# zsyOAOA/ResShift

Measured on AMD Instinct MI355X. Metric: images/sec (1x3x64x64 LR -> 3x256x256, 15-step ResShift sampling loop incl. VQ encode/decode), higher is better.
Workload: dtype f16x2 encoder + UNet (hi+lo fp16 pairs, 3 MFMAs per product: fp32-class) + f16 decoder (parity policy); 1 GPU; realsr_swinunet_realesrgan256: batch 32/GPU x 1 GPU, 1x3x64x64 LR -> 3x256x256, 15 steps, random-init weights; precision_policy=parity, parallelism=dp1 (batch sharded, one RCCL weight broadcast, no data-path collective)

## Files before the change

resshift_amd/csrc/ops.hip:

```cpp
#include "launchers.h"
#include "weight_pack.h"
#include <algorithm>
#include <cmath>
#include <cstdio>
#include <cstdlib>
#include <vector>

extern "C" {

static void* dev_copy(const void* host, size_t bytes) {
    void* d = nullptr;
    if (hipMalloc(&d, bytes) != hipSuccess) return nullptr;
    (void)hipMemcpy(d, host, bytes, hipMemcpyHostToDevice);
    return d;
}
static void* frag_major_from_device_rows(const void* wdev, int N, int K, int ld, int lo_off) {
    std::vector<f16> rows((size_t)N * ld), out((size_t)N * K * (lo_off >= 0 ? 2 : 1));
    if (hipMemcpy(rows.data(), wdev, rows.size() * sizeof(f16), hipMemcpyDeviceToHost) != hipSuccess) return nullptr;
    frag_major_fill(N, K, out.data(), lo_off >= 0, [&](int n, int k) { return rows[(size_t)n * ld + k]; },
                    [&](int n, int k) { return rows[(size_t)n * ld + (lo_off >= 0 ? lo_off : 0) + k]; });
    return dev_copy(out.data(), out.size() * sizeof(f16));
}
static void* pack_rows_dev(const float* w_ref_host, int Cout, int Cin, int taps, int prec) {
    std::vector<char> o((size_t)Cout * taps * Cin * rs_dtype_size(prec));
    if (prec == RS_F16) rs_pack_rows_f16(w_ref_host, Cout, Cin, taps, Cin, (f16*)o.data());
    else if (prec == RS_F16S) rs_pack_rows_split(w_ref_host, Cout, Cin, taps, Cin, (f16*)o.data());
    else rs_pack_rows_f32(w_ref_host, Cout, Cin, taps, Cin, (float*)o.data());
    return dev_copy(o.data(), o.size());
}
static void bias_tables_dev(const float* table_host, int heads, float** bias_t, float** bias_n, float** bias_c) {
    std::vector<float> bt(bias_t ? (size_t)heads * 4096 : 0), bn(bias_n ? (size_t)heads * 4096 : 0), bc(bias_c ? (size_t)heads * 256 : 0);
    rs_pack_bias_tables(table_host, heads, bias_t ? bt.data() : nullptr, bias_n ? bn.data() : nullptr);
    if (bias_c) rs_pack_bias_compact(table_host, heads, bc.data());
    if (bias_t) *bias_t = (float*)dev_copy(bt.data(), bt.size() * 4);
    if (bias_n) *bias_n = (float*)dev_copy(bn.data(), bn.size() * 4);
    if (bias_c) *bias_c = (float*)dev_copy(bc.data(), bc.size() * 4);
}

static int time_launches(const IGemmParams& p, int in_prec, int out_prec, const ConvPlan& pl, int reps, hipStream_t st, float* ms_out) {
    int rc = 0;
    hipEvent_t e0, e1;
    (void)hipEventCreate(&e0); (void)hipEventCreate(&e1);
    (void)hipEventRecord(e0, st);
    for (int i = 0; i < reps; ++i) rc |= rs_conv_launch(&p, in_prec, out_prec, 1, &pl, st);
    (void)hipEventRecord(e1, st);
    (void)hipEventSynchronize(e1);
    float ms = 0.f;
    (void)hipEventElapsedTime(&ms, e0, e1);
    if (ms_out) *ms_out = ms / (float)std::max(1, reps);
    (void)hipEventDestroy(e0); (void)hipEventDestroy(e1);
    return rc;
}

static int op_conv_run(IGemmParams p, int in_prec, int out_prec, hipStream_t st, bool halo_only = false, bool timed = false, int reps = 0, float* ms_out = nullptr) {
    ConvPlan pl{};
    (void)rs_conv_plan(&p, in_prec, out_prec, 1, &pl);
    if (halo_only && pl.kernel != CK_HALO && pl.kernel != CK_HALO_SEG) return rs_set_last_error("shape is not eligible for the halo kernel", -1);
    float* part = nullptr;
    if (pl.splitk > 1) { (void)hipMalloc((void**)&part, (size_t)pl.splitk * p.M * p.Cout * sizeof(float)); p.partial = part; }
    int rc = rs_conv_launch(&p, in_prec, out_prec, 1, &pl, st);
    if (rc) rs_set_last_error("igemm launch rejected the shape", -1);
    else if (timed) rc = time_launches(p, in_prec, out_prec, pl, reps, st, ms_out);
    (void)hipStreamSynchronize(st);
    if (part) (void)hipFree(part);
    return rc;
}

int rs_op_conv2d(const void* x0, const void* x1, const float* w_ref_host, const float* bias_host, const void* res, void* y, int B, int Hs,
                 int Ws, int C0, int C1, int Cout, int KH, int KW, int stride, int pad_t, int pad_l, int Ho, int Wo, int up, int act,
                 int in_prec, int out_prec, int force_direct, void* stream) {
    hipStream_t st = (hipStream_t)stream;
    const int Cin = C0 + C1;
    const size_t K = (size_t)KH * KW * Cin, n = K * Cout;
    const bool direct = force_direct || (Cin % 8 != 0) || (C0 % 8 != 0) || Cout <= 8;
    float* bias = bias_host ? (float*)dev_copy(bias_host, Cout * 4) : nullptr;
    int rc;
    void* wdev = nullptr;
    if (direct) {
        std::vector<float> o(n);
        rs_pack_tap_major(w_ref_host, Cout, Cin, KH * KW, o.data());
        wdev = dev_copy(o.data(), n * 4);
        DirectConvParams p{};
        p.x0 = x0; p.x1 = x1; p.w = (const float*)wdev; p.bias = bias; p.y = y; p.C0 = C0; p.C1 = C1; p.ld0 = C0; p.ld1 = C1;
        p.B = B; p.Hs = Hs; p.Ws = Ws; p.up = up; p.Ho = Ho; p.Wo = Wo; p.KH = KH; p.KW = KW; p.stride = stride; p.pad_t = pad_t; p.pad_l = pad_l;
        p.Cout = Cout; p.ldy = Cout; p.act = act;
        if (res) { rc = rs_set_last_error("direct conv has no residual path", -1); }
        else rc = rs_direct_conv_launch(&p, in_prec, out_prec, st);
    } else {
        wdev = pack_rows_dev(w_ref_host, Cout, Cin, KH * KW, in_prec);
        IGemmParams p{};
        p.x0 = x0; p.x1 = x1; p.w = wdev; p.bias = bias; p.res = res; p.y = y; p.C0 = C0; p.C1 = C1; p.ld0 = C0; p.ld1 = C1;
        p.B = B; p.Hs = Hs; p.Ws = Ws; p.up = up; p.Ho = Ho; p.Wo = Wo; p.KH = KH; p.KW = KW; p.stride = stride; p.pad_t = pad_t; p.pad_l = pad_l;
        p.Cout = Cout; p.ldy = Cout; p.ldres = Cout; p.M = B * Ho * Wo; p.Ktot = (int)K; p.act = act; p.out_scale = 1.f;
        rc = op_conv_run(p, in_prec, out_prec, st);
    }
    (void)hipStreamSynchronize(st);
    if (wdev) (void)hipFree(wdev);
    if (bias) (void)hipFree(bias);
    return rc;
}

int rs_op_conv2d_bench(const void* x0, const void* w_packed_dev, const float* bias_dev, const void* res, void* y, int B, int Hs, int Ws,
                       int Cin, int Cout, int KH, int KW, int stride, int pad, int Ho, int Wo, int up, int act, int in_prec, int out_prec,
                       int reps, float* ms_out, void* stream) {
    hipStream_t st = (hipStream_t)stream;
    IGemmParams p{};
    p.x0 = x0; p.w = w_packed_dev; p.bias = bias_dev; p.res = res; p.y = y; p.C0 = Cin; p.ld0 = Cin;
    p.B = B; p.Hs = Hs; p.Ws = Ws; p.up = up; p.Ho = Ho; p.Wo = Wo; p.KH = KH; p.KW = KW; p.stride = stride; p.pad_t = pad; p.pad_l = pad;
    p.Cout = Cout; p.ldy = Cout; p.ldres = Cout; p.M = B * Ho * Wo; p.Ktot = KH * KW * Cin; p.act = act; p.out_scale = 1.f;
    return op_conv_run(p, in_prec, out_prec, st, false, true, reps, ms_out);
}

int rs_op_conv3x3_halo(const void* x, const float* coef_dev, int act_in, const float* w_ref_host, const float* bias_host, const void* res, void* y,
                       int B, int H, int W, int Cin, int Cout, int prec, float* ystats_dev, void* stream) {
    hipStream_t st = (hipStream_t)stream;
    const size_t K = (size_t)9 * Cin;
    if (prec != RS_F16 && prec != RS_F16S) return rs_set_last_error("halo kernel: fp16 or split storage", -1);
    void* wdev = pack_rows_dev(w_ref_host, Cout, Cin, 9, prec);
    float* bias = bias_host ? (float*)dev_copy(bias_host, Cout * 4) : nullptr;
    IGemmParams p{};
    p.x0 = x; p.w = wdev; p.bias = bias; p.res = res; p.y = y; p.C0 = Cin; p.ld0 = Cin; p.B = B; p.Hs = H; p.Ws = W; p.up = 1; p.Ho = H; p.Wo = W;
    p.KH = 3; p.KW = 3; p.stride = 1; p.pad_t = 1; p.pad_l = 1; p.Cout = Cout; p.ldy = Cout; p.ldres = Cout; p.M = B * H * W; p.Ktot = (int)K;
    p.out_scale = 1.f; p.splitk = 1; p.xcoef = coef_dev; p.xact = act_in;
    p.ystats = ystats_dev; p.ystats_ld = Cout;
    const int rc = op_conv_run(p, prec, prec, st, true);
    if (wdev) (void)hipFree(wdev);
    if (bias) (void)hipFree(bias);
    return rc;
}

int rs_op_conv3x3_wino(const void* x, const float* coef_dev, int act_in, const float* w_ref_host, const float* bias_host, const void* res, void* y,
                       int B, int H, int W, int Cin, int Cout, float* ystats_dev, int reps, float* ms_out, void* stream) {
    hipStream_t st = (hipStream_t)stream;
    if (Cin < 32 || (Cin % 32) || Cout < 32 || (Cout % 32)) return rs_set_last_error("wino kernel: channels in multiples of 32", -1);
    std::vector<char> packed(rs_wino_weight_bytes(Cin, Cout));
    const float mx = rs_wino_pack(w_ref_host, Cin, Cout, packed.data());
    if (!(mx < 30.0f)) return rs_set_last_error("wino kernel: |U| >= 30", -1);
    void* wdev = dev_copy(packed.data(), packed.size());
    float* bias = bias_host ? (float*)dev_copy(bias_host, Cout * 4) : nullptr;
    IGemmParams p{};
    p.x0 = x; p.ww = wdev; p.bias = bias; p.res = res; p.y = y; p.C0 = Cin; p.ld0 = Cin; p.B = B; p.Hs = H; p.Ws = W; p.up = 1; p.Ho = H; p.Wo = W;
    p.KH = 3; p.KW = 3; p.stride = 1; p.pad_t = 1; p.pad_l = 1; p.Cout = Cout; p.ldy = Cout; p.ldres = Cout; p.M = B * H * W; p.Ktot = 9 * Cin;
    p.out_scale = 1.f; p.splitk = 1; p.xcoef = coef_dev; p.xact = act_in; p.ystats = ystats_dev; p.ystats_ld = Cout;
    int rc = 0;
    float* stamps = nullptr;
    const int ntile = rs_wino_tiles(&p);
    p.dbg = 64;
    if (const char* ab = getenv("RS_WINO_ABL")) p.dbg |= atoi(ab);
    if (getenv("RS_WINO_STAMPS")) { (void)hipMalloc((void**)&stamps, (size_t)ntile * 16 * sizeof(float)); (void)hipMemset(stamps, 0, (size_t)ntile * 16 * sizeof(float)); p.partial = stamps; }
    ConvPlan pl{};
    (void)rs_conv_plan(&p, RS_F16S, RS_F16S, 1, &pl);
    if (pl.kernel != CK_WINO) rc = rs_set_last_error("shape is not eligible for the wino kernel", -1);
    else {
        rc = rs_conv_launch(&p, RS_F16S, RS_F16S, 1, &pl, st);
        if (rc) rs_set_last_error("wino launch failed", -1);
        if (stamps) {
            (void)hipStreamSynchronize(st);
            std::vector<float> hs((size_t)ntile * 16);
            (void)hipMemcpy(hs.data(), stamps, hs.size() * sizeof(float), hipMemcpyDeviceToHost);
            double wide[16] = {}; int nw = 0;
            for (int t = 0; t < ntile; ++t) {
                for (int i = 0; i < 16; ++i) wide[i] += hs[(size_t)t * 16 + i];
                ++nw;
            }
            static const char* nm[8] = {"prologue", "wait+barrier", "halo issue", "B operand", "MFMA steps", "conversion", "epilogue", "total"};
            fprintf(stderr, "[wino phases] %dx%dx%d %d->%d, mean cycles of wave 0 over %d workgroups:", B, H, W, Cin, Cout, nw);
            for (int i = 0; i < 8; ++i) fprintf(stderr, " %s %.0f", nm[i], wide[i] / std::max(1, nw));
            static const char* nq[6] = {"drain", "barrier-1", "exchange writes", "barrier-2", "transform + stores", "statistics"};
            fprintf(stderr, "  | epilogue:");
            for (int i = 0; i < 6; ++i) fprintf(stderr, " %s %.0f", nq[i], wide[8 + i] / std::max(1, nw));
            fprintf(stderr, "\n");
        }
        if (!rc && reps > 0) rc = time_launches(p, RS_F16S, RS_F16S, pl, reps, st, ms_out);
    }
    (void)hipStreamSynchronize(st);
    if (stamps) (void)hipFree(stamps);
    if (wdev) (void)hipFree(wdev);
    if (bias) (void)hipFree(bias);
    return rc;
}

int rs_op_conv3x3_halo_stats_px(int B, int H, int W, int Cin, int Cout, int prec) {
    IGemmParams p{};
    p.C0 = Cin; p.ld0 = Cin; p.B = B; p.Hs = H; p.Ws = W; p.up = 1; p.Ho = H; p.Wo = W;
    p.KH = 3; p.KW = 3; p.stride = 1; p.pad_t = 1; p.pad_l = 1; p.Cout = Cout; p.ldy = Cout; p.ldres = Cout; p.M = B * H * W; p.Ktot = 9 * Cin;
    ConvPlan pl{};
    (void)rs_conv_plan(&p, prec, prec, 1, &pl);
    return (pl.kernel == CK_HALO || pl.kernel == CK_HALO_SEG) ? pl.stats_px : 0;
}

int rs_op_gemm_nt(const void* a, const void* b, const float* bias_dev, void* y, int nz, int M, int N, int K, float scale, int in_prec,
                  int out_prec, void* stream) {
    IGemmParams p{};
    p.x0 = a; p.w = b; p.bias = bias_dev; p.y = y; p.C0 = K; p.ld0 = K; p.B = 1; p.Hs = M; p.Ws = 1; p.up = 1; p.Ho = M; p.Wo = 1;
    p.KH = 1; p.KW = 1; p.stride = 1; p.Cout = N; p.ldy = N; p.M = M; p.Ktot = K; p.out_scale = scale;
    p.bs_x0 = (long long)M * K; p.bs_w = (long long)N * K; p.bs_y = (long long)M * N;
    ConvPlan pl{};
    (void)rs_conv_plan(&p, in_prec, out_prec, nz, &pl);
    const int rc = rs_conv_launch(&p, in_prec, out_prec, nz, &pl, (hipStream_t)stream);
    if (rc) rs_set_last_error("igemm launch rejected the shape", -1);
    return rc;
}

int rs_op_groupnorm(const void* x, void* y, const float* gamma_host, const float* beta_host, const float* film_dev, int B, int HW, int C,
                    int groups, float eps, int act, int prec, void* stream) {
    hipStream_t st = (hipStream_t)stream;
    float* g = (float*)dev_copy(gamma_host, C * 4);
    float* bt = (float*)dev_copy(beta_host, C * 4);
    int S = std::max(1, std::min(64, 1024 / std::max(1, B)));
    S = std::max(1, std::min(S, HW / 8));
    const int S2 = std::max(1, std::min(HW / 8, std::max(1, 2048 / std::max(1, B))));
    float* partial = nullptr;
    (void)hipMalloc((void**)&partial, (size_t)B * S * groups * 2 * 4);
    GNParams p{};
    p.x = x; p.y = y; p.gamma = g; p.beta = bt; p.film = film_dev; p.partial = partial; p.B = B; p.HW = HW; p.C = C; p.ldx = C; p.ldy = C;
    p.S = S; p.groups = groups; p.eps = eps; p.act = act;
    const int nk = rs_groupnorm_launch(&p, prec, S2, st);
    const int rc = nk < 0 ? nk : 0;
    if (rc) rs_set_last_error("groupnorm launch rejected the shape", -1);
    (void)hipStreamSynchronize(st);
    (void)hipFree(g); (void)hipFree(bt); (void)hipFree(partial);
    return rc;
}

int rs_op_window_attention(const void* qkv, void* out, const float* table_host, int B, int H, int W, int heads, int shift, int prec,
                           void* stream) {
    hipStream_t st = (hipStream_t)stream;
    float *d = nullptr, *dn = nullptr;
    bias_tables_dev(table_host, heads, &d, &dn, nullptr);
    WinAttnParams p{};
    p.bias_n = dn;
    p.qkv = qkv; p.out = out; p.bias_t = d; p.B = B; p.H = H; p.W = W; p.heads = heads; p.shift = shift; p.ldq = 3 * heads * 32;
    p.ldo = heads * 32; p.scale = 1.0f / std::sqrt(32.0f);
    const int rc = rs_win_attn_launch(&p, prec, st);
    if (rc) rs_set_last_error("window attention launch rejected the shape", -1);
    (void)hipStreamSynchronize(st);
    (void)hipFree(d);
    (void)hipFree(dn);
    return rc;
}

static int op_window_attention_qkv(bool split, const void* x, const void* wqkv_dev, const float* bqkv_dev, const void* wproj_dev, const float* bproj_dev,
                                   const void* res, void* out, const float* table_host, const float* xcoef_dev, int B, int H, int W, int heads, int shift,
                                   hipStream_t st) {
    float *dn = nullptr, *dc = nullptr;
    bias_tables_dev(table_host, heads, nullptr, &dn, &dc);
    WinAttnParams p{};
    p.bias_n = dn; p.bias_c = dc; p.out = out; p.B = B; p.H = H; p.W = W; p.heads = heads; p.shift = shift; p.ldo = heads * 32; p.scale = 1.0f / std::sqrt(32.0f);
    const int E = heads * 32, ld = split ? 2 * E : E, lo_off = split ? E : -1;
    void* wq_f = frag_major_from_device_rows(wqkv_dev, 3 * E, E, ld, lo_off);
    void* wp_f = wproj_dev ? frag_major_from_device_rows(wproj_dev, E, E, ld, lo_off) : nullptr;
    p.x = x; p.wqkv = wq_f; p.bqkv = bqkv_dev; p.ldx = heads * 32; p.xcoef = xcoef_dev;
    p.wproj = wp_f; p.bproj = bproj_dev; p.res = res; p.ldres = heads * 32;
    const int rc = !(wq_f && (wp_f || !wproj_dev)) ? -1 : (split ? rs_win_attn_qkv_split_launch(&p, st) : rs_win_attn_qkv_launch(&p, st));
    if (rc) rs_set_last_error(split ? "fused split qkv + window attention launch rejected the shape (split storage, 6 heads of 32 only)"
                                    : "fused qkv + window attention launch rejected the shape (fp16, 6 heads of 32 only)", -1);
    (void)hipStreamSynchronize(st);
    (void)hipFree(dn); (void)hipFree(dc); (void)hipFree(wq_f); (void)hipFree(wp_f);
    return rc;
}
int rs_op_window_attention_qkv(const void* x, const void* wqkv_dev, const float* bqkv_dev, const void* wproj_dev, const float* bproj_dev,
                               const void* res, void* out, const float* table_host, int B, int H, int W, int heads, int shift, void* stream) {
    return op_window_attention_qkv(false, x, wqkv_dev, bqkv_dev, wproj_dev, bproj_dev, res, out, table_host, nullptr, B, H, W, heads, shift, (hipStream_t)stream);
}
int rs_op_window_attention_qkv_split(const void* x, const void* wqkv_dev, const float* bqkv_dev, const void* wproj_dev, const float* bproj_dev,
                                     const void* res, void* out, const float* table_host, const float* xcoef_dev, int B, int H, int W, int heads,
                                     int shift, void* stream) {
    return op_window_attention_qkv(true, x, wqkv_dev, bqkv_dev, wproj_dev, bproj_dev, res, out, table_host, xcoef_dev, B, H, W, heads, shift, (hipStream_t)stream);
}

int rs_op_ae_flash_attention(const void* q, const void* k, const void* vt, const float* bv_dev, void* o, int nz, int T, int C, void* stream) {
    const int rc = rs_ae_flash_launch(q, C, k, C, vt, bv_dev, o, C, nz, T, C, 1.0f / std::sqrt((float)C), (hipStream_t)stream);
    if (rc) rs_set_last_error("streaming AE attention launch rejected the shape (fp16, C in {128, 256, 512}, T a multiple of 128)", -1);
    return rc;
}

int rs_op_ae_flash_attention_split(const void* q, const void* k, const void* vt, const float* bv_dev, void* o, int nz, int T, int C, void* stream) {
    const int rc = rs_ae_flash_split_launch(q, C, k, C, vt, bv_dev, o, C, nz, T, C, 1.0f / std::sqrt((float)C), (hipStream_t)stream);
    if (rc) rs_set_last_error("split-storage streaming AE attention launch rejected the shape (C = 512, T a multiple of 64)", -1);
    return rc;
}

int rs_op_swin_mlp(const void* x, const void* w1_dev, const float* b1_dev, const void* w2_dev, const float* b2_dev, const void* res, void* y,
                   int M, int E, int HD, void* stream) {
    const int rc = rs_swin_mlp_launch(x, w1_dev, b1_dev, w2_dev, b2_dev, res, y, M, E, E, E, E, HD, nullptr, 0, nullptr, 0, (hipStream_t)stream);
    if (rc) rs_set_last_error("swin_mlp launch rejected the shape (fp16, E = 192, HD = 768 only)", -1);
    return rc;
}
int rs_op_swin_mlp_split(const void* x, const void* w1_dev, const float* b1_dev, const void* w2_dev, const float* b2_dev, const void* res, void* y,
                         int M, int E, int HD, void* stream) {
    const int rc = rs_swin_mlp_split_launch(x, w1_dev, b1_dev, w2_dev, b2_dev, res, y, M, E, E, E, E, HD, nullptr, 0, nullptr, 0, nullptr, (hipStream_t)stream);
    if (rc) rs_set_last_error("swin_mlp_split launch rejected the shape (split storage, E = 192, HD = 768 only)", -1);
    return rc;
}
int rs_op_swin_mlp_split_unembed(const void* x, const float* xcoef_dev, const void* w1_dev, const float* b1_dev, const void* w2cat_dev, const float* bcat_dev,
                                 void* y, int M, int HW, int E, int HD, int NO, void* stream) {
    const int rc = rs_swin_mlp_split_launch_n(x, w1_dev, b1_dev, w2cat_dev, bcat_dev, nullptr, y, M, E, 0, NO, E, HD, NO, xcoef_dev, HW, nullptr, 0, nullptr,
                                              (hipStream_t)stream);
    if (rc) rs_set_last_error("swin_mlp_split (+ patch_unembed) launch rejected the shape (split storage, E = 192, HD = 768, NO = 160, HW % 128 == 0 only)", -1);
    return rc;
}
int rs_op_softmax_rows(const float* s, void* out, long long nrows, int ncols, int out_prec, void* stream) {
    return rs_softmax_rows_launch(s, out, out_prec, nrows, ncols, ncols, ncols, (hipStream_t)stream);
}
int rs_op_vq(const float* z, const float* codebook_dev, float* zq, int32_t* idx, long long N, int NE, int D, void* stream) {
    return rs_vq_launch(z, codebook_dev, zq, idx, N, NE, D, (hipStream_t)stream);
}
int rs_op_nchw_to_nhwc(const float* in, void* out, int B, int C, int HW, int out_prec, void* stream) {
    return rs_nchw_to_nhwc_launch(in, out, out_prec, B, C, HW, C, 0, 1.f, (hipStream_t)stream);
}
int rs_op_nhwc_to_nchw(const void* in, float* out, int B, int C, int HW, int in_prec, void* stream) {
    return rs_nhwc_to_nchw_launch(in, in_prec, out, B, C, HW, C, 0, (hipStream_t)stream);
}
int rs_op_convert(const void* src, int src_prec, void* dst, int dst_prec, int C, long long npix, void* stream) {
    return rs_convert_launch(src, src_prec, dst, dst_prec, C, npix, (hipStream_t)stream);
}

}
```

resshift_amd/csrc/wino.hip:

```cpp
#include "igemm_common.h"
#include "launchers.h"
#include "gn_tail.h"
#include <algorithm>
#include <cmath>
#include <vector>

namespace {

using namespace igemm_detail;

typedef __attribute__((address_space(3))) void* lds_ptr_t;

__device__ __forceinline__ void wdma16s(__amdgpu_buffer_rsrc_t r, char* lds, unsigned voff, unsigned soff) {
    __builtin_amdgcn_raw_ptr_buffer_load_lds(r, (lds_ptr_t)lds, 16, voff, soff, 0, 0);
}

template <int N> __device__ __forceinline__ void wait_vm() { asm volatile("s_waitcnt vmcnt(%0)" ::"n"(N) : "memory"); }

constexpr int W_TH = 8, W_TW = 16;
constexpr int W_PITCH = 20;
constexpr int W_HROWS = (W_TH + 2) * W_PITCH;
constexpr int W_UPW = 2;
constexpr int W_NUNIT = 8 * W_UPW;
constexpr int W_HBUF = W_NUNIT * 2048;
constexpr int W_NBUF = 3;
constexpr int W_COEF = W_NBUF * W_HBUF;
constexpr int W_MAXCIN = 640;
constexpr int W_LDS = 160 * 1024;
static_assert(W_COEF + W_MAXCIN * 8 <= W_LDS && W_COEF + 8 * 1024 <= W_LDS, "LDS");
constexpr unsigned W_INV = 0xF0000000u;
__host__ __device__ constexpr int w_depth_of(int CF) { return CF <= 8 ? 4 : 2; }

__host__ __device__ constexpr int w_first(int i) { return i == 0 ? 0 : 1; }
__host__ __device__ constexpr int w_second(int i) { return i == 3 ? 3 : 2; }
__host__ __device__ constexpr float w_tau(int i) { return i == 1 ? 1.f : -1.f; }
__host__ __device__ constexpr float w_sigma(int i) { return i == 2 ? -1.f : 1.f; }
__host__ __device__ constexpr int w_cf_of(int Cout) { return (Cout % 160) == 0 ? 10 : ((Cout % 128) == 0 ? 8 : 4); }

#ifdef RS_WINO_PHASES
#define WSTAMP(i) do { const long long t_ = __builtin_readcyclecounter(); ph[i] += t_ - tprev; tprev = t_; } while (0)
#define WABL(bit) (p.dbg & (bit))
#else
#define WSTAMP(i) do {} while (0)
#define WABL(bit) false
#endif

template <int CF>
__global__ __launch_bounds__(512, 2) void wino_kernel(IGemmParams p) {
    constexpr int W_DEPTH = w_depth_of(CF);
    static_assert(CF % W_DEPTH == 0, "register slots for the weight fragments: the slot of a step is cf % W_DEPTH");
    constexpr int BC = 16 * CF, CFH = CF / 2;
    extern __shared__ __attribute__((aligned(16))) char smem[];
    const int tid = threadIdx.x, lane = tid & 63;
    const int wave = __builtin_amdgcn_readfirstlane(tid >> 6);
#ifdef RS_WINO_PHASES
    long long ph[16] = {0, 0, 0, 0, 0, 0, 0, 0, 0, 0, 0, 0, 0, 0, 0, 0};
    long long tprev = __builtin_readcyclecounter();
    const long long tstart = tprev;
#endif
    const int nby = p.Cout / BC;
    const int txb_n = p.Wo / W_TW, tyb_n = p.Ho / W_TH;
    int tile = xcd_remap(blockIdx.x, gridDim.x);
    const int nb = tile % nby; tile /= nby;
    const int txb = tile % txb_n; tile /= txb_n;
    const int tyb = tile % tyb_n;
    const int b = tile / tyb_n;
    const int n0 = nb * BC, y0 = tyb * W_TH, x0 = txb * W_TW;
    const int Cin = p.C0, ld0 = p.ld0, Hs = p.Hs, Ws = p.Ws;
    const int nch = Cin / 32;
    const int R = max(1, min(nch, 1024 / p.Cout));
    const int c0 = (int)((blockIdx.x >> 3) % (unsigned)R);
    auto chunk_of = [&](int c) -> int { const int t = c + c0; return t >= nch ? t - nch : t; };
    const float* const xcoef = p.xcoef;
    const int xact = p.xact;

    const __amdgpu_buffer_rsrc_t rx = __builtin_amdgcn_make_buffer_rsrc((void*)p.x0, 0, p.x_bytes, 0x00020000);

    const int pi = wave >> 1, jp = wave & 1;
    const float tau_a = w_tau(pi);
    const int pflip = (int)((blockIdx.x >> 3) / (unsigned)max(1, min(p.C0 / 32, 1024 / p.Cout))) & 1;
    const float tau_b[2] = {w_tau(2 * jp + pflip), w_tau(2 * jp + (1 ^ pflip))};
    const int a1 = w_first(pi), a2 = w_second(pi);

    auto row_src = [&](int row, unsigned& pix) -> bool {
        const int hy = row / W_PITCH, sx = row - hy * W_PITCH;
        const int hx = sx < 10 ? 2 * sx : 2 * (sx - 10) + 1;
        const int y = y0 - 1 + hy, x = x0 - 1 + hx;
        pix = (unsigned)((b * Hs + y) * Ws + x);
        return row < W_HROWS && hx < 18 && (unsigned)y < (unsigned)Hs && (unsigned)x < (unsigned)Ws;
    };
    unsigned xv[W_UPW][2];
#pragma unroll
    for (int k = 0; k < W_UPW; ++k)
#pragma unroll
        for (int h = 0; h < 2; ++h) {
            const int unit = wave + 8 * k, row = 16 * unit + 8 * h + (lane >> 3), slot = lane & 7;
            const int g = (slot >> 1) ^ ((row >> 1) & 3);
            unsigned pix;
            const bool ok = row_src(row, pix);
            xv[k][h] = ok ? pix * (unsigned)ld0 * 4u + (unsigned)(slot & 1) * (unsigned)ld0 * 2u + (unsigned)g * 16u : W_INV;
        }
    auto issue_halo = [&](int c, int buf) __attribute__((always_inline)) {
        char* hb = smem + buf * W_HBUF;
        const bool live = c < nch;
#pragma unroll
        for (int k = 0; k < W_UPW; ++k)
#pragma unroll
            for (int h = 0; h < 2; ++h) wdma16s(rx, hb + (wave + 8 * k) * 2048 + h * 1024, live ? xv[k][h] : W_INV, (unsigned)(live ? chunk_of(c) : 0) * 64u);
    };
    unsigned in_mask = 0;
#pragma unroll
    for (int k = 0; k < W_UPW; ++k) {
        unsigned pix;
        if (row_src(16 * (wave + 8 * k) + (lane >> 2), pix)) in_mask |= 1u << k;
    }
    const int cv_g = (lane & 3) ^ (((lane >> 2) >> 1) & 3);
    const float* const coefs = (const float*)(smem + W_COEF);
    auto convert = [&](int c, int buf, auto act_tag) __attribute__((always_inline)) {
        constexpr int ACT = decltype(act_tag)::value;
        f32x4 ca0 = {1.f, 1.f, 1.f, 1.f}, ca1 = ca0, cd0 = {0.f, 0.f, 0.f, 0.f}, cd1 = cd0;
        if (xcoef) {
            const float* sc = coefs + chunk_of(c) * 32 + cv_g * 8;
            ca0 = *(const f32x4*)sc; ca1 = *(const f32x4*)(sc + 4); cd0 = *(const f32x4*)(sc + Cin); cd1 = *(const f32x4*)(sc + Cin + 4);
        }
        char* hb = smem + buf * W_HBUF + lane * 32;
#pragma unroll
        for (int k = 0; k < W_UPW; ++k) {
            const bool in = (in_mask >> k) & 1;
            char* cell = hb + (wave + 8 * k) * 2048;
            const f16x8 vh = *(const f16x8*)cell, vl = *(const f16x8*)(cell + 16);
            f32x4 o0, o1;
#pragma unroll
            for (int e = 0; e < 8; ++e) {
                const float t = fmaf(rs_join(vh[e], vl[e]), e < 4 ? ca0[e & 3] : ca1[e & 3], e < 4 ? cd0[e & 3] : cd1[e & 3]);
                float u = ACT == RS_ACT_SILU ? t * __builtin_amdgcn_rcpf(1.0f + __expf(-t)) : t;
                u = in ? u : 0.f;
                if (e < 4) o0[e & 3] = u; else o1[e & 3] = u;
            }
            *(f32x4*)cell = o0; *(f32x4*)(cell + 16) = o1;
        }
    };
    auto convert_chunk = [&](int c, int buf) __attribute__((always_inline)) {
        if (xact == RS_ACT_SILU) convert(c, buf, std::integral_constant<int, RS_ACT_SILU>{});
        else convert(c, buf, std::integral_constant<int, RS_ACT_NONE>{});
    };

    const char* const wbase = (const char*)p.ww + ((size_t)nb * 16u + (size_t)(4 * pi + 2 * jp)) * (size_t)nch * (size_t)CF * 2048u;
    const int wpos_step = nch * CF * 2048;
    const int wvl = lane * 16;
    auto load_w = [&](int c, int pp, int cf, int ds, f16x8& h, f16x8& l) __attribute__((always_inline)) {
        const int t = pp * CF + cf + ds, q = t / CF;
        const int cc = chunk_of(min(c + (q >> 1), nch - 1));
        const char* src = wbase + ((q & 1) ^ pflip) * wpos_step + (cc * CF + t % CF) * 2048 + wvl;
        h = *(const f16x8*)src; l = *(const f16x8*)(src + 1024);
    };

    int ax[2][4];
    {
        const int tx = lane & 7, tyl = (lane >> 3) & 1, g = lane >> 4;
#pragma unroll
        for (int pp = 0; pp < 2; ++pp) {
            const int j = 2 * jp + (pp ^ pflip), b1 = w_first(j), b2 = w_second(j);
#pragma unroll
            for (int k = 0; k < 4; ++k) {
                const int a = (k & 2) ? a2 : a1, bb = (k & 1) ? b2 : b1;
                const int r = (2 * tyl + a) * W_PITCH + tx + (bb >> 1) + 10 * (bb & 1);
                ax[pp][k] = r * 128 + ((g ^ ((r >> 1) & 3)) << 5) + ((g & 1) << 4);
            }
        }
    }
    auto make_b = [&](int pp, int tf, f16x8& h, f16x8& l) __attribute__((always_inline)) {
        const char* q = smem + tf * (4 * W_PITCH * 128);
        const float tb = tau_b[pp];
#pragma unroll
        for (int half = 0; half < 2; ++half) {
            f32x4 px[4];
#pragma unroll
            for (int k = 0; k < 4; ++k) px[k] = *(const f32x4*)(q + (half ? (ax[pp][k] ^ 16) : ax[pp][k]));
#pragma unroll
            for (int e = 0; e < 4; ++e) {
                const float v = fmaf(fmaf(px[3][e], tb, px[2][e]), tau_a, fmaf(px[1][e], tb, px[0][e]));
                f16 hh, ll;
                rs_split(v, hh, ll); h[4 * half + e] = hh; l[4 * half + e] = ll;
            }
        }
    };

    f32x4 acc[2][2][CF];
#pragma unroll
    for (int pp = 0; pp < 2; ++pp)
#pragma unroll
        for (int tf = 0; tf < 2; ++tf)
#pragma unroll
            for (int i = 0; i < CF; ++i) acc[pp][tf][i] = f32x4{0.f, 0.f, 0.f, 0.f};

    if (xcoef) {
        const __amdgpu_buffer_rsrc_t rc = __builtin_amdgcn_make_buffer_rsrc((void*)(xcoef + (long long)b * 2 * Cin), 0, 2 * Cin * 4, 0x00020000);
        wdma16s(rc, smem + W_COEF + wave * 1024, (unsigned)(wave * 1024 + lane * 16), 0u);
    }
    issue_halo(0, 0);
    issue_halo(1, 1);
    f16x8 wh[W_DEPTH], wl[W_DEPTH];
    __builtin_amdgcn_sched_barrier(0);
#pragma unroll
    for (int s = 0; s < W_DEPTH; ++s) load_w(0, 0, 0, s, wh[s], wl[s]);
    __builtin_amdgcn_sched_barrier(0);
    wait_vm<2 * W_UPW + 2 * W_DEPTH>();
    asm volatile("s_waitcnt lgkmcnt(0)" ::: "memory");
    __builtin_amdgcn_s_barrier();
    asm volatile("" ::: "memory");
    convert_chunk(0, 0);
    WSTAMP(0);

    int buf = 0;
    for (int c = 0; c < nch; ++c) {
        wait_vm<2 * W_DEPTH>();
        asm volatile("s_waitcnt lgkmcnt(0)" ::: "memory");
        __builtin_amdgcn_s_barrier();
        asm volatile("" ::: "memory");
        WSTAMP(1);
        const int buf1 = buf == 2 ? 0 : buf + 1, buf2 = buf1 == 2 ? 0 : buf1 + 1;
        issue_halo(c + 2, buf2);
        WSTAMP(2);
#pragma unroll
        for (int pp = 0; pp < 2; ++pp) {
            f16x8 bh[2], bl[2];
            if (WABL(2)) { bh[0] = bh[1] = bl[0] = bl[1] = wh[0]; }
            else {
#pragma unroll
                for (int tf = 0; tf < 2; ++tf) { make_b(pp, tf, bh[tf], bl[tf]); __builtin_amdgcn_sched_barrier(0); }
            }
            WSTAMP(3);
#pragma unroll
            for (int cf = 0; cf < CF; ++cf) {
                const f16x8 ah = wh[cf % W_DEPTH], al = wl[cf % W_DEPTH];
                const f16x8 as = ah * (f16)RS_LO_SCALE;
                if (WABL(1)) { acc[pp][0][cf][0] += (float)(as[0] * bh[0][0] + al[1] * bl[1][1]); }
                else {
#pragma unroll
                    for (int tf = 0; tf < 2; ++tf) acc[pp][tf][cf] = __builtin_amdgcn_mfma_f32_16x16x32_f16(as, bh[tf], acc[pp][tf][cf], 0, 0, 0);
#pragma unroll
                    for (int tf = 0; tf < 2; ++tf) acc[pp][tf][cf] = __builtin_amdgcn_mfma_f32_16x16x32_f16(ah, bl[tf], acc[pp][tf][cf], 0, 0, 0);
#pragma unroll
                    for (int tf = 0; tf < 2; ++tf) acc[pp][tf][cf] = __builtin_amdgcn_mfma_f32_16x16x32_f16(al, bh[tf], acc[pp][tf][cf], 0, 0, 0);
                }
                __builtin_amdgcn_sched_barrier(0);
                if (!WABL(8)) load_w(c, pp, cf, W_DEPTH, wh[cf % W_DEPTH], wl[cf % W_DEPTH]);
                __builtin_amdgcn_sched_barrier(0);
            }
            WSTAMP(4);
        }
        if (c + 1 < nch && !WABL(4)) convert_chunk(c + 1, buf1);
        WSTAMP(5);
        {
            const int flip = buf == 2 ? -2 * W_HBUF : W_HBUF;
#pragma unroll
            for (int pp = 0; pp < 2; ++pp)
#pragma unroll
                for (int k = 0; k < 4; ++k) ax[pp][k] += flip;
        }
        buf = buf1;
    }

    constexpr int TS = CFH * 64 + 16;
    constexpr int NO = 2 * CFH;
    constexpr int NITEM = 16 * NO * 2;
    static_assert(16 * 16 * TS <= W_LDS && NITEM <= 512, "exchange");
    const float osc = p.out_scale * RS_LO_INV;
    float* const ystats = p.ystats;
    const bool tail_on = p.tail.coef != nullptr;
    const f16* res = (const f16*)p.res;
    f16* y = (f16*)p.y;
    const int ldres = p.ldres, ldy = p.ldy;
    const bool item = tid < NITEM;
    const int oct = tid % NO, tl = (tid / NO) & 15, yy = item ? tid / (16 * NO) : 0;
    const float sy = yy ? -1.f : 1.f;
    asm volatile("s_waitcnt vmcnt(0)" ::: "memory");
#ifdef RS_WINO_PHASES
    { const long long t_ = __builtin_readcyclecounter(); ph[8] += t_ - tprev; }
    long long tq = __builtin_readcyclecounter();
#define WQ(i) do { const long long t_ = __builtin_readcyclecounter(); ph[i] += t_ - tq; tq = t_; } while (0)
#else
#define WQ(i) do {} while (0)
#endif
    if (!WABL(16)) {
#pragma unroll
    for (int half = 0; half < 2; ++half) {
        const int nc = n0 + half * CFH * 16 + oct * 8;
        f32x4 bv0 = {0.f, 0.f, 0.f, 0.f}, bv1 = bv0;
        if (p.bias && item) { bv0 = *(const f32x4*)(p.bias + nc); bv1 = *(const f32x4*)(p.bias + nc + 4); }
        float s1[8], s2[8];
#pragma unroll
        for (int e = 0; e < 8; ++e) s1[e] = s2[e] = 0.f;
#pragma unroll
        for (int tf = 0; tf < 2; ++tf) {
            asm volatile("s_waitcnt lgkmcnt(0)" ::: "memory");
            __builtin_amdgcn_s_barrier();
            asm volatile("" ::: "memory");
            WQ(9);
#pragma unroll
            for (int pp = 0; pp < 2; ++pp)
#pragma unroll
                for (int cq = 0; cq < CFH; ++cq)
                    *(f32x4*)(smem + ((4 * pi + 2 * jp + (pp ^ pflip)) * 16 + (lane & 15)) * TS + (cq * 16 + 4 * (lane >> 4)) * 4) = acc[pp][tf][half * CFH + cq];
            const int ty = 2 * tf + ((tl >> 3) & 1), tx = tl & 7;
            const long long m0 = ((long long)b * p.Ho + y0 + 2 * ty + yy) * p.Wo + x0 + 2 * tx;
            uint4 rh[2] = {uint4{0u, 0u, 0u, 0u}, uint4{0u, 0u, 0u, 0u}}, rl[2] = {uint4{0u, 0u, 0u, 0u}, uint4{0u, 0u, 0u, 0u}};
            if (res && item) {
#pragma unroll
                for (int x = 0; x < 2; ++x) {
                    const f16* rp = res + (m0 + x) * ldres * 2 + nc;
                    rh[x] = *(const uint4*)rp; rl[x] = *(const uint4*)(rp + ldres);
                }
            }
            WQ(10);
            asm volatile("s_waitcnt lgkmcnt(0)" ::: "memory");
            __builtin_amdgcn_s_barrier();
            asm volatile("" ::: "memory");
            WQ(11);
            if (item) {
                f32x4 Y0a = {0.f, 0.f, 0.f, 0.f}, Y0b = Y0a, Y1a = Y0a, Y1b = Y0a;
#pragma unroll
                for (int r = 0; r < 3; ++r) {
                    const char* base = smem + (((yy + r) * 4) * 16 + tl) * TS + oct * 32;
                    f32x4 ma[4], mb[4];
#pragma unroll
                    for (int j = 0; j < 4; ++j) { ma[j] = *(const f32x4*)(base + j * 16 * TS); mb[j] = *(const f32x4*)(base + j * 16 * TS + 16); }
                    const f32x4 r0a = ma[0] + ma[1] + ma[2], r0b = mb[0] + mb[1] + mb[2];
                    const f32x4 r1a = ma[1] - ma[2] - ma[3], r1b = mb[1] - mb[2] - mb[3];
                    const float sg = r == 0 ? 1.f : sy;
                    Y0a += r0a * sg; Y0b += r0b * sg; Y1a += r1a * sg; Y1b += r1b * sg;
                }
#pragma unroll
                for (int x = 0; x < 2; ++x) {
                    const f32x4 va = (x ? Y1a : Y0a) * osc + bv0, vb = (x ? Y1b : Y0b) * osc + bv1;
                    float v[8] = {va[0], va[1], va[2], va[3], vb[0], vb[1], vb[2], vb[3]};
                    if (res) {
                        const f16x8 h8 = __builtin_bit_cast(f16x8, rh[x]), l8 = __builtin_bit_cast(f16x8, rl[x]);
#pragma unroll
                        for (int e = 0; e < 8; ++e) v[e] += rs_join(h8[e], l8[e]);
                    }
                    f16x8 oh, ol;
#pragma unroll
                    for (int e = 0; e < 8; ++e) {
                        f16 hh, ll;
                        rs_split(v[e], hh, ll); oh[e] = hh; ol[e] = ll;
                        s1[e] += v[e]; s2[e] = fmaf(v[e], v[e], s2[e]);
                    }
                    f16* yp = y + (m0 + x) * ldy * 2 + nc;
                    *(f16x8*)yp = oh; *(f16x8*)(yp + ldy) = ol;
                }
            }
            WQ(12);
        }
        if (ystats) {
            asm volatile("s_waitcnt lgkmcnt(0)" ::: "memory");
            __builtin_amdgcn_s_barrier();
            asm volatile("" ::: "memory");
            float* sb = (float*)smem;
            if (item) {
                *(f32x4*)(sb + tid * 16) = f32x4{s1[0], s1[1], s1[2], s1[3]}; *(f32x4*)(sb + tid * 16 + 4) = f32x4{s1[4], s1[5], s1[6], s1[7]};
                *(f32x4*)(sb + tid * 16 + 8) = f32x4{s2[0], s2[1], s2[2], s2[3]}; *(f32x4*)(sb + tid * 16 + 12) = f32x4{s2[4], s2[5], s2[6], s2[7]};
            }
            asm volatile("s_waitcnt lgkmcnt(0)" ::: "memory");
            __builtin_amdgcn_s_barrier();
            asm volatile("" ::: "memory");
            float* sb2 = sb + 512 * 16;
            if (tid < NO * 8 * 4) {
                const int part = tid / (NO * 8), ch = tid - part * (NO * 8);
                const int o = ch >> 3, e = ch & 7;
                float a = 0.f, q = 0.f;
#pragma unroll
                for (int k = 8 * part; k < 8 * part + 8; ++k) { a += sb[(o + NO * k) * 16 + e]; q += sb[(o + NO * k) * 16 + 8 + e]; }
                sb2[(part * NO * 8 + ch) * 2] = a; sb2[(part * NO * 8 + ch) * 2 + 1] = q;
            }
            asm volatile("s_waitcnt lgkmcnt(0)" ::: "memory");
            __builtin_amdgcn_s_barrier();
            asm volatile("" ::: "memory");
            if (tid < NO * 8) {
                float a = 0.f, q = 0.f;
#pragma unroll
                for (int part = 0; part < 4; ++part) { a += sb2[(part * NO * 8 + tid) * 2]; q += sb2[(part * NO * 8 + tid) * 2 + 1]; }
                float* dst = ystats + (((long long)b * (tyb_n * txb_n) + tyb * txb_n + txb) * p.ystats_ld + n0 + half * CFH * 16 + tid) * 2;
                if (tail_on) rs_pub_pair(dst, a, q);
                else { dst[0] = a; dst[1] = q; }
            }
            WQ(13);
        }
    }
    if (ystats && tail_on) {
        asm volatile("s_waitcnt vmcnt(0)" ::: "memory");
        __syncthreads();
        unsigned* const tail_flag = (unsigned*)(smem + 65536);
        if (wave == 0) { const bool last = rs_gn_tail_arrive(p.tail, b); if (lane == 0) *tail_flag = last ? 1u : 0u; }
        __syncthreads();
        if (*tail_flag) rs_gn_tail_finish<512>(p.tail, b, (float*)smem);
    }
    }
#ifdef RS_WINO_PHASES
    WSTAMP(6);
    ph[7] = tprev - tstart;
    if (tid == 0 && p.partial) {
#pragma unroll
        for (int i = 0; i < 16; ++i) p.partial[(size_t)blockIdx.x * 16 + i] = (float)ph[i];
    }
#endif
}

template <int CF> hipError_t wino_launch_cf(const IGemmParams& p, int tiles, hipStream_t st) {
    static RsAttrFlags attr_flags;
    if (attr_flags.need()) (void)hipFuncSetAttribute((const void*)wino_kernel<CF>, hipFuncAttributeMaxDynamicSharedMemorySize, W_LDS);
    hipLaunchKernelGGL((wino_kernel<CF>), dim3(tiles), dim3(512), W_LDS, st, p);
    return hipGetLastError();
}

}

extern "C" size_t rs_wino_weight_bytes(int Cin, int Cout) { return (size_t)Cin * Cout * 64; }

extern "C" float rs_wino_pack(const float* w, int Cin, int Cout, void* dst_) {
    f16* dst = (f16*)dst_;
    static const double G[4][3] = {{1, 0, 0}, {.5, .5, .5}, {.5, -.5, .5}, {0, 0, 1}};
    const int nch = Cin / 32, CF = w_cf_of(Cout), BC = 16 * CF;
    float mx = 0.f;
    for (int n = 0; n < Cout; ++n) {
        const int nb = n / BC, nl = n - nb * BC, cf = nl / 16, lr = nl & 15;
        const size_t blk = (size_t)nb * 16 * nch * CF * 1024;
        for (int ci = 0; ci < Cin; ++ci) {
            const float* g9 = w + ((size_t)n * Cin + ci) * 9;
            double t[4][3];
            for (int i = 0; i < 4; ++i)
                for (int k = 0; k < 3; ++k) t[i][k] = G[i][0] * g9[0 * 3 + k] + G[i][1] * g9[1 * 3 + k] + G[i][2] * g9[2 * 3 + k];
            const int c = ci / 32, g = (ci % 32) / 8, e0 = ci % 8;
            const int e = (g & 1) ? ((e0 + 4) & 7) : e0;
            const int lane = g * 16 + lr;
            for (int i = 0; i < 4; ++i)
                for (int j = 0; j < 4; ++j) {
                    const double u = (t[i][0] * G[j][0] + t[i][1] * G[j][1] + t[i][2] * G[j][2]) * (double)(w_sigma(i) * w_sigma(j));
                    const float uf = (float)u;
                    mx = std::max(mx, std::fabs(uf));
                    f16 h, l;
                    rs_split(uf, h, l);
                    const size_t o = blk + ((((size_t)(4 * i + j) * nch + c) * CF + cf) * 2) * 512 + (size_t)lane * 8 + e;
                    dst[o] = h; dst[o + 512] = l;
                }
        }
    }
    return mx;
}

extern "C" int rs_wino_plan(const IGemmParams* pp, int in_dt, int out_dt, int nz, ConvPlan* pl) {
    static const int on = []() { const char* e = getenv("RS_WINO"); return e ? atoi(e) : 1; }();
    static const int min_tiles = []() { const char* e = getenv("RS_WINO_MINTILES"); return e ? atoi(e) : 192; }();
    const IGemmParams& p = *pp;
    if (!on || in_dt != RS_F16S || out_dt != RS_F16S || nz != 1 || !p.ww || p.C1 != 0 || p.unscaled_w || p.sC || p.act != RS_ACT_NONE) return 0;
    if (p.KH != 3 || p.KW != 3 || p.stride != 1 || p.pad_t != 1 || p.pad_l != 1 || p.up != 1 || p.Ho != p.Hs || p.Wo != p.Ws || p.osc == 2) return 0;
    if ((p.C0 % 32) || p.C0 > W_MAXCIN || (p.ld0 % 8) || (p.Cout % (16 * w_cf_of(p.Cout))) || (p.ldy % 8) || (p.res && (p.ldres % 8))) return 0;
    if ((p.Ho % W_TH) || (p.Wo % W_TW)) return 0;
    const long long tiles = (long long)p.B * (p.Ho / W_TH) * (p.Wo / W_TW) * (p.Cout / (16 * w_cf_of(p.Cout)));
    if (tiles < min_tiles && !(p.dbg & 64)) return 0;
    *pl = ConvPlan{CK_WINO, W_TH * W_TW, 16 * w_cf_of(p.Cout), 0, 1, W_TH * W_TW};
    return 1;
}

extern "C" int rs_wino_tiles(const IGemmParams* p) { return p->B * (p->Ho / W_TH) * (p->Wo / W_TW) * (p->Cout / (16 * w_cf_of(p->Cout))); }

extern "C" int rs_wino_launch(const IGemmParams* pp, hipStream_t st) {
    IGemmParams p = *pp;
    if (((size_t)p.x0 & 15) || ((size_t)p.y & 15) || ((size_t)p.res & 15) || ((size_t)p.ww & 15)) return -2;
    const size_t xb = (size_t)p.B * p.Hs * p.Ws * p.ld0 * 4;
    if (xb >= 0xF0000000ull) return -2;
    p.x_bytes = (unsigned)xb;
    const int CF = w_cf_of(p.Cout), nby = p.Cout / (16 * CF), per_image = (p.Ho / W_TH) * (p.Wo / W_TW);
    if (p.tail.coef) {
        if (!p.ystats) return -2;
        if (p.tail.C > 2048 || p.tail.groups < 1 || p.tail.groups > 64 || (p.tail.C % p.tail.groups)) return -2;
        p.tail.expected = per_image * nby;
        p.tail.st0 = p.ystats; p.tail.S0 = per_image; p.tail.ld0 = p.ystats_ld; p.tail.n0 = p.Cout;
    }
    const int tiles = p.B * per_image * nby;
    const hipError_t e = CF == 10 ? wino_launch_cf<10>(p, tiles, st) : (CF == 8 ? wino_launch_cf<8>(p, tiles, st) : wino_launch_cf<4>(p, tiles, st));
    return e == hipSuccess ? 0 : -1;
}
```

Baseline: 133.0 images/sec.

## Restructure Winograd epilogue into double-buffered rounds with pipelined statistics

The Winograd conv epilogue is rewritten so every thread owns one output pixel and an 8-channel octet, and processes channel rounds of 32. Each round's exchange is double-buffered in LDS, and the next round's write overlaps the current round's output transform. The group-norm statistics are reduced with DPP cross-lane shuffles and their partial and total sums are spread over later rounds, which removes the separate barrier-heavy statistics phase. Bias is staged in LDS and residuals are loaded up front, which costs more registers and a new LDS layout with swizzled addresses.

```diff
diff --git a/resshift_amd/csrc/ops.hip b/resshift_amd/csrc/ops.hip
--- a/resshift_amd/csrc/ops.hip
+++ b/resshift_amd/csrc/ops.hip
@@ -164,9 +164,9 @@
                 ++nw;
             }
             static const char* nm[8] = {"prologue", "wait+barrier", "halo issue", "B operand", "MFMA steps", "conversion", "epilogue", "total"};
-            fprintf(stderr, "[wino phases] %dx%dx%d %d->%d, mean cycles of wave 0 over %d workgroups:", B, H, W, Cin, Cout, nw);
+            fprintf(stderr, "[wino phases] %dx%dx%d %d->%d, mean cycles of the stamped wave over %d workgroups:", B, H, W, Cin, Cout, nw);
             for (int i = 0; i < 8; ++i) fprintf(stderr, " %s %.0f", nm[i], wide[i] / std::max(1, nw));
-            static const char* nq[6] = {"drain", "barrier-1", "exchange writes", "barrier-2", "transform + stores", "statistics"};
+            static const char* nq[6] = {"drain", "barriers", "exchange writes", "statistics in rounds", "transform + stores", "statistics tail"};
             fprintf(stderr, "  | epilogue:");
             for (int i = 0; i < 6; ++i) fprintf(stderr, " %s %.0f", nq[i], wide[8 + i] / std::max(1, nw));
             fprintf(stderr, "\n");
diff --git a/resshift_amd/csrc/wino.hip b/resshift_amd/csrc/wino.hip
--- a/resshift_amd/csrc/wino.hip
+++ b/resshift_amd/csrc/wino.hip
@@ -38,6 +38,9 @@
 __host__ __device__ constexpr int w_cf_of(int Cout) { return (Cout % 160) == 0 ? 10 : ((Cout % 128) == 0 ? 8 : 4); }
 
 #ifdef RS_WINO_PHASES
+#ifndef RS_WINO_PHASE_WAVE
+#define RS_WINO_PHASE_WAVE 0
+#endif
 #define WSTAMP(i) do { const long long t_ = __builtin_readcyclecounter(); ph[i] += t_ - tprev; tprev = t_; } while (0)
 #define WABL(bit) (p.dbg & (bit))
 #else
@@ -49,7 +52,7 @@
 __global__ __launch_bounds__(512, 2) void wino_kernel(IGemmParams p) {
     constexpr int W_DEPTH = w_depth_of(CF);
     static_assert(CF % W_DEPTH == 0, "register slots for the weight fragments: the slot of a step is cf % W_DEPTH");
-    constexpr int BC = 16 * CF, CFH = CF / 2;
+    constexpr int BC = 16 * CF;
     extern __shared__ __attribute__((aligned(16))) char smem[];
     const int tid = threadIdx.x, lane = tid & 63;
     const int wave = __builtin_amdgcn_readfirstlane(tid >> 6);
@@ -262,19 +265,29 @@
         buf = buf1;
     }
 
-    constexpr int TS = CFH * 64 + 16;
-    constexpr int NO = 2 * CFH;
-    constexpr int NITEM = 16 * NO * 2;
-    static_assert(16 * 16 * TS <= W_LDS && NITEM <= 512, "exchange");
+    constexpr int NR = CF / 2;
+    constexpr int X_TFS = 8 * 2048 + 128;
+    constexpr int X_XS = 2 * X_TFS + 64;
+    constexpr int X_BUF = 2 * X_XS;
+    constexpr int X_PARK = 2 * X_BUF;
+    constexpr int X_SB2 = X_PARK + 2 * 8192;
+    constexpr int X_BIAS = X_SB2 + 2 * 1024;
+    static_assert(X_BIAS >= W_COEF + 8 * 1024 && X_BIAS + BC * 4 <= W_LDS && (CF % 2) == 0, "exchange");
+    {
     const float osc = p.out_scale * RS_LO_INV;
     float* const ystats = p.ystats;
     const bool tail_on = p.tail.coef != nullptr;
     const f16* res = (const f16*)p.res;
     f16* y = (f16*)p.y;
     const int ldres = p.ldres, ldy = p.ldy;
-    const bool item = tid < NITEM;
-    const int oct = tid % NO, tl = (tid / NO) & 15, yy = item ? tid / (16 * NO) : 0;
+    const int oct = tid & 3, ox = (tid >> 2) & 1, otf = (tid >> 3) & 1, yy = (tid >> 4) & 1, tyl = (tid >> 5) & 1, tx = wave;
     const float sy = yy ? -1.f : 1.f;
+    const long long m0 = ((long long)b * p.Ho + y0 + 4 * otf + 2 * tyl + yy) * p.Wo + x0 + 2 * tx + ox;
+    const int nc0 = n0 + oct * 8;
+    const char* const rd = smem + ox * X_XS + otf * X_TFS + (2 * yy) * 2048 + (tyl * 8 + tx) * 128;
+    const int rs0 = (oct ^ tx) << 4, rs1 = rs0 ^ 64;
+    char* const wr = smem + (2 * pi + jp) * 2048 + (lane & 15) * 128;
+    const int ws0 = ((((lane >> 4) & 1) * 4 + (lane >> 5)) ^ (lane & 7)) << 4, ws1 = ws0 ^ 32;
     asm volatile("s_waitcnt vmcnt(0)" ::: "memory");
 #ifdef RS_WINO_PHASES
     { const long long t_ = __builtin_readcyclecounter(); ph[8] += t_ - tprev; }
@@ -284,109 +297,127 @@
 #define WQ(i) do {} while (0)
 #endif
     if (!WABL(16)) {
-#pragma unroll
-    for (int half = 0; half < 2; ++half) {
-        const int nc = n0 + half * CFH * 16 + oct * 8;
+    float* const xbias = (float*)(smem + X_BIAS);
+    if (p.bias && tid < BC / 4) *(f32x4*)(xbias + 4 * tid) = *(const f32x4*)(p.bias + n0 + 4 * tid);
+    uint4 rh[NR], rl[NR];
+#pragma unroll
+    for (int r = 0; r < NR; ++r) {
+        rh[r] = rl[r] = uint4{0u, 0u, 0u, 0u};
+        if (res) {
+            const f16* rp = res + m0 * ldres * 2 + nc0 + 32 * r;
+            rh[r] = *(const uint4*)rp; rl[r] = *(const uint4*)(rp + ldres);
+        }
+    }
+    auto xbarrier = [&]() __attribute__((always_inline)) {
+        asm volatile("s_waitcnt lgkmcnt(0)" ::: "memory");
+        __builtin_amdgcn_s_barrier();
+        asm volatile("" ::: "memory");
+    };
+    const int off_s = jp ? X_XS : 0, off_m = jp ? 0 : X_XS;
+    const float sg_s = jp ? -1.f : 1.f;
+    const bool m_is_1 = (pflip != 0) != (jp == 0);
+    auto xwrite = [&](int r) __attribute__((always_inline)) {
+        char* w = wr + (r & 1) * X_BUF;
+#pragma unroll
+        for (int tf = 0; tf < 2; ++tf)
+#pragma unroll
+            for (int f = 0; f < 2; ++f) {
+                const f32x4 a0 = acc[0][tf][2 * r + f], a1 = acc[1][tf][2 * r + f];
+                *(f32x4*)(w + off_s + tf * X_TFS + (f ? ws1 : ws0)) = (a0 + a1) * sg_s;
+                *(f32x4*)(w + off_m + tf * X_TFS + (f ? ws1 : ws0)) = m_is_1 ? a1 : a0;
+            }
+    };
+    float* const park = (float*)(smem + X_PARK);
+    float* const sb2 = (float*)(smem + X_SB2);
+    auto part_sums = [&](int r) __attribute__((always_inline)) {
+        if (tid < 128) {
+            const int ch = tid & 31, part = tid >> 5;
+            const float* src = park + (((r & 1) * 4 + part) * 8) * 64 + (ch >> 3) * 16 + (ch & 7);
+            float a = 0.f, q = 0.f;
+#pragma unroll
+            for (int k = 0; k < 8; ++k) { a += src[k * 64]; q += src[k * 64 + 8]; }
+            sb2[(((r & 1) * 4 + part) * 32 + ch) * 2] = a; sb2[(((r & 1) * 4 + part) * 32 + ch) * 2 + 1] = q;
+        }
+    };
+    auto totals = [&](int r) __attribute__((always_inline)) {
+        if (tid < 32) {
+            float a = 0.f, q = 0.f;
+#pragma unroll
+            for (int part = 0; part < 4; ++part) { a += sb2[(((r & 1) * 4 + part) * 32 + tid) * 2]; q += sb2[(((r & 1) * 4 + part) * 32 + tid) * 2 + 1]; }
+            float* dst = ystats + (((long long)b * (tyb_n * txb_n) + tyb * txb_n + txb) * p.ystats_ld + n0 + 32 * r + tid) * 2;
+            if (tail_on) rs_pub_pair(dst, a, q);
+            else { dst[0] = a; dst[1] = q; }
+        }
+    };
+    xbarrier();
+    WQ(9);
+    xwrite(0);
+    WQ(10);
+#pragma unroll
+    for (int r = 0; r < NR; ++r) {
+        xbarrier();
+        WQ(9);
+        if (ystats) {
+            if (r >= 1) part_sums(r - 1);
+            if (r >= 2) totals(r - 2);
+        }
+        WQ(11);
+        const int nc = nc0 + 32 * r;
         f32x4 bv0 = {0.f, 0.f, 0.f, 0.f}, bv1 = bv0;
-        if (p.bias && item) { bv0 = *(const f32x4*)(p.bias + nc); bv1 = *(const f32x4*)(p.bias + nc + 4); }
-        float s1[8], s2[8];
-#pragma unroll
-        for (int e = 0; e < 8; ++e) s1[e] = s2[e] = 0.f;
-#pragma unroll
-        for (int tf = 0; tf < 2; ++tf) {
-            asm volatile("s_waitcnt lgkmcnt(0)" ::: "memory");
-            __builtin_amdgcn_s_barrier();
-            asm volatile("" ::: "memory");
-            WQ(9);
-#pragma unroll
-            for (int pp = 0; pp < 2; ++pp)
-#pragma unroll
-                for (int cq = 0; cq < CFH; ++cq)
-                    *(f32x4*)(smem + ((4 * pi + 2 * jp + (pp ^ pflip)) * 16 + (lane & 15)) * TS + (cq * 16 + 4 * (lane >> 4)) * 4) = acc[pp][tf][half * CFH + cq];
-            const int ty = 2 * tf + ((tl >> 3) & 1), tx = tl & 7;
-            const long long m0 = ((long long)b * p.Ho + y0 + 2 * ty + yy) * p.Wo + x0 + 2 * tx;
-            uint4 rh[2] = {uint4{0u, 0u, 0u, 0u}, uint4{0u, 0u, 0u, 0u}}, rl[2] = {uint4{0u, 0u, 0u, 0u}, uint4{0u, 0u, 0u, 0u}};
-            if (res && item) {
-#pragma unroll
-                for (int x = 0; x < 2; ++x) {
-                    const f16* rp = res + (m0 + x) * ldres * 2 + nc;
-                    rh[x] = *(const uint4*)rp; rl[x] = *(const uint4*)(rp + ldres);
-                }
-            }
-            WQ(10);
-            asm volatile("s_waitcnt lgkmcnt(0)" ::: "memory");
-            __builtin_amdgcn_s_barrier();
-            asm volatile("" ::: "memory");
-            WQ(11);
-            if (item) {
-                f32x4 Y0a = {0.f, 0.f, 0.f, 0.f}, Y0b = Y0a, Y1a = Y0a, Y1b = Y0a;
-#pragma unroll
-                for (int r = 0; r < 3; ++r) {
-                    const char* base = smem + (((yy + r) * 4) * 16 + tl) * TS + oct * 32;
-                    f32x4 ma[4], mb[4];
-#pragma unroll
-                    for (int j = 0; j < 4; ++j) { ma[j] = *(const f32x4*)(base + j * 16 * TS); mb[j] = *(const f32x4*)(base + j * 16 * TS + 16); }
-                    const f32x4 r0a = ma[0] + ma[1] + ma[2], r0b = mb[0] + mb[1] + mb[2];
-                    const f32x4 r1a = ma[1] - ma[2] - ma[3], r1b = mb[1] - mb[2] - mb[3];
-                    const float sg = r == 0 ? 1.f : sy;
-                    Y0a += r0a * sg; Y0b += r0b * sg; Y1a += r1a * sg; Y1b += r1b * sg;
-                }
-#pragma unroll
-                for (int x = 0; x < 2; ++x) {
-                    const f32x4 va = (x ? Y1a : Y0a) * osc + bv0, vb = (x ? Y1b : Y0b) * osc + bv1;
-                    float v[8] = {va[0], va[1], va[2], va[3], vb[0], vb[1], vb[2], vb[3]};
-                    if (res) {
-                        const f16x8 h8 = __builtin_bit_cast(f16x8, rh[x]), l8 = __builtin_bit_cast(f16x8, rl[x]);
-#pragma unroll
-                        for (int e = 0; e < 8; ++e) v[e] += rs_join(h8[e], l8[e]);
-                    }
-                    f16x8 oh, ol;
-#pragma unroll
-                    for (int e = 0; e < 8; ++e) {
-                        f16 hh, ll;
-                        rs_split(v[e], hh, ll); oh[e] = hh; ol[e] = ll;
-                        s1[e] += v[e]; s2[e] = fmaf(v[e], v[e], s2[e]);
-                    }
-                    f16* yp = y + (m0 + x) * ldy * 2 + nc;
-                    *(f16x8*)yp = oh; *(f16x8*)(yp + ldy) = ol;
-                }
-            }
-            WQ(12);
-        }
+        if (p.bias) { bv0 = *(const f32x4*)(xbias + nc - n0); bv1 = *(const f32x4*)(xbias + nc - n0 + 4); }
+        f32x4 Ya = {0.f, 0.f, 0.f, 0.f}, Yb = Ya;
+        {
+            const char* base = rd + (r & 1) * X_BUF;
+#pragma unroll
+            for (int i = 0; i < 3; ++i) {
+                const f32x4 v0a = *(const f32x4*)(base + (2 * i) * 2048 + rs0), v0b = *(const f32x4*)(base + (2 * i) * 2048 + rs1);
+                const f32x4 v1a = *(const f32x4*)(base + (2 * i + 1) * 2048 + rs0), v1b = *(const f32x4*)(base + (2 * i + 1) * 2048 + rs1);
+                const float sg = i == 0 ? 1.f : sy;
+                Ya += (v0a + v1a) * sg; Yb += (v0b + v1b) * sg;
+            }
+        }
+        if (r + 1 < NR) xwrite(r + 1);
+        const f32x4 va = Ya * osc + bv0, vb = Yb * osc + bv1;
+        float v[8] = {va[0], va[1], va[2], va[3], vb[0], vb[1], vb[2], vb[3]};
+        if (res) {
+            const f16x8 h8 = __builtin_bit_cast(f16x8, rh[r]), l8 = __builtin_bit_cast(f16x8, rl[r]);
+#pragma unroll
+            for (int e = 0; e < 8; ++e) v[e] += rs_join(h8[e], l8[e]);
+        }
+        f16x8 oh, ol;
+#pragma unroll
+        for (int e = 0; e < 8; ++e) {
+            f16 hh, ll;
+            rs_split(v[e], hh, ll); oh[e] = hh; ol[e] = ll;
+        }
+        f16* yp = y + m0 * ldy * 2 + nc;
+        *(f16x8*)yp = oh; *(f16x8*)(yp + ldy) = ol;
         if (ystats) {
-            asm volatile("s_waitcnt lgkmcnt(0)" ::: "memory");
-            __builtin_amdgcn_s_barrier();
-            asm volatile("" ::: "memory");
-            float* sb = (float*)smem;
-            if (item) {
-                *(f32x4*)(sb + tid * 16) = f32x4{s1[0], s1[1], s1[2], s1[3]}; *(f32x4*)(sb + tid * 16 + 4) = f32x4{s1[4], s1[5], s1[6], s1[7]};
-                *(f32x4*)(sb + tid * 16 + 8) = f32x4{s2[0], s2[1], s2[2], s2[3]}; *(f32x4*)(sb + tid * 16 + 12) = f32x4{s2[4], s2[5], s2[6], s2[7]};
-            }
-            asm volatile("s_waitcnt lgkmcnt(0)" ::: "memory");
-            __builtin_amdgcn_s_barrier();
-            asm volatile("" ::: "memory");
-            float* sb2 = sb + 512 * 16;
-            if (tid < NO * 8 * 4) {
-                const int part = tid / (NO * 8), ch = tid - part * (NO * 8);
-                const int o = ch >> 3, e = ch & 7;
-                float a = 0.f, q = 0.f;
-#pragma unroll
-                for (int k = 8 * part; k < 8 * part + 8; ++k) { a += sb[(o + NO * k) * 16 + e]; q += sb[(o + NO * k) * 16 + 8 + e]; }
-                sb2[(part * NO * 8 + ch) * 2] = a; sb2[(part * NO * 8 + ch) * 2 + 1] = q;
-            }
-            asm volatile("s_waitcnt lgkmcnt(0)" ::: "memory");
-            __builtin_amdgcn_s_barrier();
-            asm volatile("" ::: "memory");
-            if (tid < NO * 8) {
-                float a = 0.f, q = 0.f;
-#pragma unroll
-                for (int part = 0; part < 4; ++part) { a += sb2[(part * NO * 8 + tid) * 2]; q += sb2[(part * NO * 8 + tid) * 2 + 1]; }
-                float* dst = ystats + (((long long)b * (tyb_n * txb_n) + tyb * txb_n + txb) * p.ystats_ld + n0 + half * CFH * 16 + tid) * 2;
-                if (tail_on) rs_pub_pair(dst, a, q);
-                else { dst[0] = a; dst[1] = q; }
-            }
-            WQ(13);
-        }
+            float s1[8], s2[8];
+#pragma unroll
+            for (int e = 0; e < 8; ++e) {
+                const int vi = __float_as_int(v[e]);
+                const float v1 = __int_as_float(__builtin_amdgcn_update_dpp(vi, vi, 0x12C, 0xF, 0xF, false));
+                const float v2 = __int_as_float(__builtin_amdgcn_update_dpp(vi, vi, 0x128, 0xF, 0xF, false));
+                const float v3 = __int_as_float(__builtin_amdgcn_update_dpp(vi, vi, 0x124, 0xF, 0xF, false));
+                s1[e] = 0.f; s1[e] += v[e]; s1[e] += v1; s1[e] += v2; s1[e] += v3;
+                s2[e] = fmaf(v3, v3, fmaf(v2, v2, fmaf(v1, v1, fmaf(v[e], v[e], 0.f))));
+            }
+            if ((tid & 12) == 0) {
+                float* dstp = park + ((((r & 1) * 4 + 2 * yy + tyl) * 8 + tx) * 4 + oct) * 16;
+                *(f32x4*)dstp = f32x4{s1[0], s1[1], s1[2], s1[3]}; *(f32x4*)(dstp + 4) = f32x4{s1[4], s1[5], s1[6], s1[7]};
+                *(f32x4*)(dstp + 8) = f32x4{s2[0], s2[1], s2[2], s2[3]}; *(f32x4*)(dstp + 12) = f32x4{s2[4], s2[5], s2[6], s2[7]};
+            }
+        }
+        WQ(12);
+    }
+    if (ystats) {
+        xbarrier();
+        part_sums(NR - 1);
+        if (NR >= 2) totals(NR - 2);
+        xbarrier();
+        totals(NR - 1);
+        WQ(13);
     }
     if (ystats && tail_on) {
         asm volatile("s_waitcnt vmcnt(0)" ::: "memory");
@@ -397,10 +428,11 @@
         if (*tail_flag) rs_gn_tail_finish<512>(p.tail, b, (float*)smem);
     }
     }
+    }
 #ifdef RS_WINO_PHASES
     WSTAMP(6);
     ph[7] = tprev - tstart;
-    if (tid == 0 && p.partial) {
+    if (tid == 64 * RS_WINO_PHASE_WAVE && p.partial) {
 #pragma unroll
         for (int i = 0; i < 16; ++i) p.partial[(size_t)blockIdx.x * 16 + i] = (float)ph[i];
     }
```

New measurement: 134.1 images/sec (median of 6 runs). About the same (+0.8%).
